# PrimeIntellect-ai/pi-quant

Measured on AMD Instinct MI355X. Metric: GiB/s quantize fp32->uint8 (numel=27.26M, nearest), higher is better.
Workload: dtype f32

## Files before the change

pi-quant_amd/csrc/quant_kernels.hpp:

```cpp
#pragma once

#include <cstdio>
#include <cstdlib>

#include "device_math.hpp"
#include "stop_event.hpp"

namespace pq {

typedef uint32_t u32x4 __attribute__((ext_vector_type(4)));
typedef uint32_t u32x2 __attribute__((ext_vector_type(2)));

enum : int { ST_PLAIN = 0, ST_NT = 1, ST_WT = 2 };
constexpr int mem_policy(bool nt_loads, int store_policy) { return (nt_loads ? 1 : 0) | (store_policy << 1); }

template <bool NT, typename T>
__device__ __forceinline__ T ld(const T* p) {
    typedef T unaligned_t __attribute__((aligned(1)));
    const unaligned_t* q = reinterpret_cast<const unaligned_t*>(p);
    if constexpr (NT) return __builtin_nontemporal_load(q);
    else return *q;
}

template <int POLICY, typename T>
__device__ __forceinline__ void st(T* p, T v) {
    typedef T unaligned_t __attribute__((aligned(1)));
    if constexpr (POLICY == ST_NT) {
        __builtin_nontemporal_store(v, reinterpret_cast<unaligned_t*>(p));
    } else if constexpr (POLICY == ST_WT) {
        if constexpr (sizeof(T) == 16) asm volatile("global_store_dwordx4 %0, %1, off sc0 sc1\n\ts_nop 1" ::"v"(p), "v"(v) : "memory");
        else if constexpr (sizeof(T) == 8) asm volatile("global_store_dwordx2 %0, %1, off sc0 sc1\n\ts_nop 0" ::"v"(p), "v"(v) : "memory");
        else if constexpr (sizeof(T) == 4) asm volatile("global_store_dword %0, %1, off sc0 sc1" ::"v"(p), "v"(v) : "memory");
        else if constexpr (sizeof(T) == 2) asm volatile("global_store_short %0, %1, off sc0 sc1" ::"v"(p), "v"(static_cast<uint32_t>(v)) : "memory");
        else asm volatile("global_store_byte %0, %1, off sc0 sc1" ::"v"(p), "v"(static_cast<uint32_t>(v)) : "memory");
    } else {
        *reinterpret_cast<unaligned_t*>(p) = v;
    }
}

template <int DT_IN>
struct InVec {
    static constexpr int EPV = DT_IN == DT_F32 ? 4 : 8;
    static __device__ __forceinline__ void unpack(const u32x4& raw, float (&v)[EPV]) {
        if constexpr (DT_IN == DT_F32) {
#pragma unroll
            for (int e = 0; e < 4; ++e) v[e] = __uint_as_float(raw[e]);
        } else {
#pragma unroll
            for (int e = 0; e < 4; ++e) {
                v[2 * e] = __uint_as_float(raw[e] << 16);
                v[2 * e + 1] = __uint_as_float(raw[e] & 0xffff0000u);
            }
        }
    }
    static __device__ __forceinline__ float load_scalar(const void* in, int64_t i) {
        if constexpr (DT_IN == DT_F32) return static_cast<const float*>(in)[i];
        else return bf16_bits_to_f32(static_cast<const uint16_t*>(in)[i]);
    }
};

template <int BITS>
struct QuantRefBlock {
    static constexpr int value = BITS == 8 ? 64 : 16;
};

template <int DT_IN, int BITS, int MODE>
__device__ __forceinline__ void quantize_bytes_guarded(const void* in, uint8_t* out, int64_t numel, int64_t byte_begin,
                                                       int64_t byte_end, const QuantParams& p, int64_t tid,
                                                       int64_t nthreads) {
    constexpr int PACK = 8 / BITS;
    constexpr int QMAX = (1 << BITS) - 1;
    for (int64_t b = byte_begin + tid; b < byte_end; b += nthreads) {
        [[maybe_unused]] RefPart part {};
        if constexpr (MODE == RM_NEAREST_FAST) {
            if (p.ref.on) part = ref_part<PACK, QuantRefBlock<BITS>::value>(p.ref, ref_partition_index<PACK>(p.ref, p.ref.index0 + b * PACK));
        }
        uint32_t acc = 0;
#pragma unroll
        for (int k = 0; k < PACK; ++k) {
            const int64_t i = b * PACK + k;
            if (i >= numel) continue;
            const float x = InVec<DT_IN>::load_scalar(in, i);
            uint32_t q;
            bool scalar_form = false;
            if constexpr (MODE == RM_NEAREST_FAST) {
                const int64_t g = p.ref.index0 + i;
                scalar_form = p.ref.on && (g < part.head_end || g >= part.body_end);
            }
            if (scalar_form) q = quant_nearest_tail32<QMAX>(x, p);
            else q = quant_one<MODE, QMAX>(x, p, static_cast<uint64_t>(i));
            acc |= q << (k * BITS);
        }
        out[b] = static_cast<uint8_t>(acc);
    }
}

template <int DT_IN, int BITS, int MODE>
__global__ void __launch_bounds__(256) quantize_scalar_kernel(const void* in, uint8_t* out, int64_t numel, QuantParams p_arg) {
    const QuantParams p = resolved(p_arg);
    constexpr int PACK = 8 / BITS;
    const int64_t nbytes = (numel + PACK - 1) / PACK;
    quantize_bytes_guarded<DT_IN, BITS, MODE>(in, out, numel, 0, nbytes, p,
                                              static_cast<int64_t>(blockIdx.x) * blockDim.x + threadIdx.x,
                                              static_cast<int64_t>(gridDim.x) * blockDim.x);
}

template <int DT_IN, int BITS, int MODE>
__device__ __forceinline__ void quantize_vec(const u32x4& raw, const QuantParams& p, const ElementKeys& keys, uint64_t e0,
                                             uint32_t (&w)[(InVec<DT_IN>::EPV * BITS / 8) > 4 ? 2 : 1]) {
    constexpr int EPV = InVec<DT_IN>::EPV, QMAX = (1 << BITS) - 1, WORDS = (EPV * BITS / 8) > 4 ? 2 : 1;
    float v[EPV];
    InVec<DT_IN>::unpack(raw, v);
#pragma unroll
    for (int j = 0; j < WORDS; ++j) w[j] = 0;
    if constexpr (MODE == RM_NEAREST_FAST) {
#pragma unroll
        for (int e = 0; e < EPV; e += 2) {
            uint32_t q0, q1;
            quant_nearest_fast2<QMAX>(v[e], v[e + 1], p, q0, q1);
            w[(e * BITS) >> 5] |= (q0 | (q1 << BITS)) << ((e * BITS) & 31);
        }
    } else if constexpr (MODE == RM_STOCH_ELEM) {
#pragma unroll
        for (int e = 0; e < EPV; ++e) {
            const uint32_t q = quant_stochastic<QMAX>(v[e], p, element_threshold(keys, p.index_base + e0 + e));
            w[(e * BITS) >> 5] |= q << ((e * BITS) & 31);
        }
    } else {
#pragma unroll
        for (int e = 0; e < EPV; ++e) {
            const uint32_t q = quant_one<MODE, QMAX>(v[e], p, e0 + e);
            w[(e * BITS) >> 5] |= q << ((e * BITS) & 31);
        }
    }
}

__device__ __forceinline__ uint32_t bfi32(uint32_t mask, uint32_t a, uint32_t b) { return (a & mask) | (b & ~mask); }

template <int EPV>
__device__ __forceinline__ void pack_saturated_u8(const float (&tz)[EPV], uint32_t (&w)[EPV / 4]) {
#pragma unroll
    for (int j = 0; j < EPV / 4; ++j) {
        uint32_t acc = 0;
#pragma unroll
        for (int e = 0; e < 4; ++e) acc = __builtin_amdgcn_cvt_pk_u8_f32(tz[j * 4 + e], static_cast<uint32_t>(e), acc);
        w[j] = acc;
    }
}

template <int BITS, int EPV>
__device__ __forceinline__ void pack_normalised(const float (&tn)[EPV], uint32_t (&w)[(EPV * BITS / 8) > 4 ? 2 : 1]) {
    auto P = [](float a, float b) -> uint32_t {
        typedef unsigned short u16x2 __attribute__((ext_vector_type(2)));
        const u16x2 r = __builtin_amdgcn_cvt_pknorm_u16(a, b);
        return __builtin_bit_cast(uint32_t, r);
    };
    constexpr uint32_t LOW_BYTES = 0x06040200u;
    static_assert(BITS == 4 || BITS == 2, "8-bit outputs gain nothing from the normalised domain (one v_perm per four elements against nothing): pack_saturated_u8");
    if constexpr (BITS == 4) {
        if constexpr (EPV == 8) {
            const uint32_t even = __builtin_amdgcn_perm(P(tn[4], tn[6]), P(tn[0], tn[2]), LOW_BYTES);
            const uint32_t odd = __builtin_amdgcn_perm(P(tn[5], tn[7]), P(tn[1], tn[3]), LOW_BYTES);
            w[0] = bfi32(0x0f0f0f0fu, even, odd);
        } else {
            const uint32_t m = bfi32(0x0f0f0f0fu, P(tn[0], tn[2]), P(tn[1], tn[3]));
            w[0] = __builtin_amdgcn_perm(0u, m, 0x0c0c0200u);
        }
    } else {
        if constexpr (EPV == 8) {
            const uint32_t t1 = bfi32(0x33333333u, P(tn[0], tn[4]), P(tn[1], tn[5]));
            const uint32_t t2 = bfi32(0x33333333u, P(tn[2], tn[6]), P(tn[3], tn[7]));
            const uint32_t u = bfi32(0x0f0f0f0fu, t1, t2);
            w[0] = __builtin_amdgcn_perm(0u, u, 0x0c0c0200u);
        } else {
            const uint32_t t = bfi32(0x33333333u, P(tn[0], tn[2]), P(tn[1], tn[3]));
            w[0] = bfi32(0x0fu, t, t >> 16) & 0xffu;
        }
    }
}

template <int N>
__device__ __forceinline__ void add_half_abs_round_down(const float (&r)[N], float (&out)[N]) {
    static_assert(N == 4, "the generic step exists for fp32 inputs only: four elements per vector");
    asm volatile("s_setreg_imm32_b32 hwreg(HW_REG_MODE, 0, 2), 2\n"
                 "v_add_f32_e64 %0, |%4|, 0.5\nv_add_f32_e64 %1, |%5|, 0.5\nv_add_f32_e64 %2, |%6|, 0.5\nv_add_f32_e64 %3, |%7|, 0.5\n"
                 "s_setreg_imm32_b32 hwreg(HW_REG_MODE, 0, 2), 0"
                 : "=&v"(out[0]), "=&v"(out[1]), "=&v"(out[2]), "=&v"(out[3])
                 : "v"(r[0]), "v"(r[1]), "v"(r[2]), "v"(r[3]));
}

template <int BITS, int EPV>
__device__ __forceinline__ void clamp_and_pack(const float (&s)[EPV], const BoundedStep& b, uint32_t (&w)[(EPV * BITS / 8) > 4 ? 2 : 1]) {
#pragma clang fp contract(off)
    constexpr float R = 1.0f / static_cast<float>((1 << BITS) - 1);
    float tz[EPV];
#pragma unroll
    for (int e = 0; e < EPV; e += 2) {
        const f32x2 pair = {s[e], s[e + 1]};
        f32x2 sum;
        if constexpr (BITS == 8) sum = pair + b.zp_float;
        else sum = __builtin_elementwise_fma(pair, f32x2 {R, R}, f32x2 {b.zp_norm, b.zp_norm});
        tz[e] = sum[0];
        tz[e + 1] = sum[1];
    }
    if constexpr (BITS == 8) pack_saturated_u8<EPV>(tz, w);
    else pack_normalised<BITS, EPV>(tz, w);
}

template <int DT_IN, int BITS, bool GENERIC = false>
__device__ __forceinline__ void quantize_vec_bounded(const u32x4& raw, float inv_scale, const BoundedStep& b,
                                                     uint32_t (&w)[(InVec<DT_IN>::EPV * BITS / 8) > 4 ? 2 : 1]) {
#pragma clang fp contract(off)
    constexpr int EPV = InVec<DT_IN>::EPV;
    float v[EPV];
    InVec<DT_IN>::unpack(raw, v);
    float t[EPV];
    if constexpr (GENERIC) {
        float prods[EPV], sums[EPV];
#pragma unroll
        for (int e = 0; e < EPV; e += 2) {
            const f32x2 x = {v[e], v[e + 1]};
            const f32x2 prod = x * inv_scale;
            prods[e] = prod[0];
            prods[e + 1] = prod[1];
        }
        add_half_abs_round_down<EPV>(prods, sums);
#pragma unroll
        for (int e = 0; e < EPV; ++e) t[e] = __builtin_copysignf(__builtin_floorf(sums[e]), prods[e]);
    } else {
#pragma unroll
        for (int e = 0; e < EPV; e += 2) {
            const f32x2 x = {v[e], v[e + 1]};
            const f32x2 prod = x * inv_scale;
            const f32x2 half = {__builtin_copysignf(0.5f, prod[0]), __builtin_copysignf(0.5f, prod[1])};
            const f32x2 adj = prod + half;
            t[e] = __builtin_truncf(adj[0]);
            t[e + 1] = __builtin_truncf(adj[1]);
        }
    }
    clamp_and_pack<BITS, EPV>(t, b, w);
}

template <int N, bool UNIFORM>
__device__ __forceinline__ void sub_abs_round_up(const float (&r)[N], const float (&t)[N], float (&out)[N]) {
    static_assert(N == 4 || N == 8, "one 16-byte vector of fp32 or bf16");
#define PQ_RU_ON "s_setreg_imm32_b32 hwreg(HW_REG_MODE, 0, 2), 1\n"
#define PQ_RU_OFF "s_setreg_imm32_b32 hwreg(HW_REG_MODE, 0, 2), 0"
    if constexpr (N == 4 && UNIFORM) {
        asm volatile(PQ_RU_ON "v_sub_f32_e64 %0, |%4|, %8\nv_sub_f32_e64 %1, |%5|, %8\nv_sub_f32_e64 %2, |%6|, %8\nv_sub_f32_e64 %3, |%7|, %8\n" PQ_RU_OFF
                     : "=&v"(out[0]), "=&v"(out[1]), "=&v"(out[2]), "=&v"(out[3])
                     : "v"(r[0]), "v"(r[1]), "v"(r[2]), "v"(r[3]), "v"(t[0]));
    } else if constexpr (N == 4) {
        asm volatile(PQ_RU_ON "v_sub_f32_e64 %0, |%4|, %8\nv_sub_f32_e64 %1, |%5|, %9\nv_sub_f32_e64 %2, |%6|, %10\nv_sub_f32_e64 %3, |%7|, %11\n" PQ_RU_OFF
                     : "=&v"(out[0]), "=&v"(out[1]), "=&v"(out[2]), "=&v"(out[3])
                     : "v"(r[0]), "v"(r[1]), "v"(r[2]), "v"(r[3]), "v"(t[0]), "v"(t[1]), "v"(t[2]), "v"(t[3]));
    } else if constexpr (UNIFORM) {
        asm volatile(PQ_RU_ON "v_sub_f32_e64 %0, |%8|, %16\nv_sub_f32_e64 %1, |%9|, %16\nv_sub_f32_e64 %2, |%10|, %16\nv_sub_f32_e64 %3, |%11|, %16\n"
                     "v_sub_f32_e64 %4, |%12|, %16\nv_sub_f32_e64 %5, |%13|, %16\nv_sub_f32_e64 %6, |%14|, %16\nv_sub_f32_e64 %7, |%15|, %16\n" PQ_RU_OFF
                     : "=&v"(out[0]), "=&v"(out[1]), "=&v"(out[2]), "=&v"(out[3]), "=&v"(out[4]), "=&v"(out[5]), "=&v"(out[6]), "=&v"(out[7])
                     : "v"(r[0]), "v"(r[1]), "v"(r[2]), "v"(r[3]), "v"(r[4]), "v"(r[5]), "v"(r[6]), "v"(r[7]), "v"(t[0]));
    } else {
        asm volatile(PQ_RU_ON "v_sub_f32_e64 %0, |%8|, %16\nv_sub_f32_e64 %1, |%9|, %17\nv_sub_f32_e64 %2, |%10|, %18\nv_sub_f32_e64 %3, |%11|, %19\n"
                     "v_sub_f32_e64 %4, |%12|, %20\nv_sub_f32_e64 %5, |%13|, %21\nv_sub_f32_e64 %6, |%14|, %22\nv_sub_f32_e64 %7, |%15|, %23\n" PQ_RU_OFF
                     : "=&v"(out[0]), "=&v"(out[1]), "=&v"(out[2]), "=&v"(out[3]), "=&v"(out[4]), "=&v"(out[5]), "=&v"(out[6]), "=&v"(out[7])
                     : "v"(r[0]), "v"(r[1]), "v"(r[2]), "v"(r[3]), "v"(r[4]), "v"(r[5]), "v"(r[6]), "v"(r[7]), "v"(t[0]), "v"(t[1]), "v"(t[2]), "v"(t[3]), "v"(t[4]),
                       "v"(t[5]), "v"(t[6]), "v"(t[7]));
    }
#undef PQ_RU_ON
#undef PQ_RU_OFF
}

template <int DT_IN, int BITS, int MODE>
__device__ __forceinline__ void quantize_vec_bounded_stochastic(const u32x4& raw, const QuantParams& p, const ElementKeys& keys, uint64_t e0,
                                                                const BoundedStep& b, uint32_t (&w)[(InVec<DT_IN>::EPV * BITS / 8) > 4 ? 2 : 1]) {
#pragma clang fp contract(off)
    static_assert(MODE == RM_STOCH_CALL || MODE == RM_STOCH_ELEM, "stochastic modes only");
    constexpr int EPV = InVec<DT_IN>::EPV;
    float v[EPV];
    InVec<DT_IN>::unpack(raw, v);
    float s[EPV], r[EPV], tau[EPV], a[EPV];
#pragma unroll
    for (int e = 0; e < EPV; e += 2) {
        const f32x2 x = {v[e], v[e + 1]};
        const f32x2 prod = x * p.inv_scale;
        r[e] = prod[0];
        r[e + 1] = prod[1];
    }
#pragma unroll
    for (int e = 0; e < EPV; ++e) tau[e] = MODE == RM_STOCH_ELEM ? element_threshold(keys, p.index_base + e0 + e) : p.threshold;
    sub_abs_round_up<EPV, MODE == RM_STOCH_CALL>(r, tau, a);
#pragma unroll
    for (int e = 0; e < EPV; ++e) s[e] = __builtin_copysignf(__builtin_ceilf(a[e]), r[e]);
    clamp_and_pack<BITS, EPV>(s, b, w);
}

template <int DT_IN, int BITS, int MODE>
__device__ __forceinline__ void quantize_vec_short(const u32x4& raw, const QuantParams& p, const ElementKeys& keys, uint64_t e0, const BoundedStep& b,
                                                   uint32_t (&w)[(InVec<DT_IN>::EPV * BITS / 8) > 4 ? 2 : 1]) {
    if constexpr (MODE == RM_NEAREST_FAST || MODE == RM_NEAREST_I64) quantize_vec_bounded<DT_IN, BITS, MODE == RM_NEAREST_I64>(raw, p.inv_scale, b, w);
    else quantize_vec_bounded_stochastic<DT_IN, BITS, MODE>(raw, p, keys, e0, b, w);
}

template <int BITS>
__device__ __forceinline__ BoundedStep bounded_step_for(int32_t zp32) {
    constexpr float QMAX = static_cast<float>((1 << BITS) - 1);
    return BoundedStep {static_cast<float>(zp32), (static_cast<float>(zp32) + 0.3f * QMAX / 65535.0f) * (1.0f / QMAX)};
}

__device__ __forceinline__ float vec_absmax_f32(const u32x4& raw, float m, bool& nan) {
#pragma unroll
    for (int e = 0; e < 4; e += 2) {
        const float a = __uint_as_float(raw[e]), b = __uint_as_float(raw[e + 1]);
        m = __builtin_fmaxf(__builtin_fmaxf(__builtin_fabsf(a), __builtin_fabsf(b)), m);
        nan |= __builtin_isunordered(a, b);
    }
    return m;
}

typedef uint16_t u16x2 __attribute__((ext_vector_type(2)));
__device__ __forceinline__ uint32_t vec_absmax_bits_bf16(const u32x4& raw, uint32_t m) {
#pragma unroll
    for (int e = 0; e < 4; ++e)
        m = __builtin_bit_cast(uint32_t, __builtin_elementwise_max(__builtin_bit_cast(u16x2, m), __builtin_bit_cast(u16x2, raw[e] & 0x7fff7fffu)));
    return m;
}
__device__ __forceinline__ float absmax_bits_to_float(uint32_t m) { return __uint_as_float(max(m & 0xffffu, m >> 16) << 16); }

template <int OB, int POLICY>
__device__ __forceinline__ void store_packed(uint8_t* dst, const uint32_t (&w)[OB > 4 ? 2 : 1]) {
    if constexpr (OB == 1) st<POLICY>(dst, static_cast<uint8_t>(w[0]));
    else if constexpr (OB == 2) st<POLICY>(reinterpret_cast<uint16_t*>(dst), static_cast<uint16_t>(w[0]));
    else if constexpr (OB == 4) st<POLICY>(reinterpret_cast<uint32_t*>(dst), w[0]);
    else st<POLICY>(reinterpret_cast<u32x2*>(dst), u32x2 {w[0], w[1]});
}

struct QuantKernargs {
    const void* in;
    uint8_t* out;
    int64_t numel;
    uint64_t ref_m;
    float inv_scale;
    int32_t zp32;
    const ParamRecord* dyn;
    uint32_t flags, look_w;
    QuantParams p;
};
constexpr uint32_t kQuantKernargRef = static_cast<uint32_t>(__builtin_offsetof(QuantKernargs, p) + __builtin_offsetof(QuantParams, ref));

template <int DT_IN, int BITS, int U, int BLOCK>
struct QuantTile {
    static constexpr int EPV = InVec<DT_IN>::EPV;
    static constexpr int OB = EPV * BITS / 8;
    static constexpr int WAVES = BLOCK / 64;
    static constexpr int WAVE_VECS = U * 64;
    static constexpr int WAVE_OUT_BYTES = WAVE_VECS * OB;
    static constexpr int LANE_OUT_BYTES = U * OB;
    static constexpr int64_t BLOCK_ELEMS = static_cast<int64_t>(WAVES) * WAVE_VECS * EPV;
};

template <int DT_IN, int BITS, int MODE, int U, bool STAGE, int NT, int BLOCK>
__global__ void __launch_bounds__(BLOCK)
quantize_kernel(const void* __restrict__ in, uint8_t* __restrict__ out, int64_t numel, uint64_t look_m, float inv_scale, int32_t zp32,
                const ParamRecord* dyn, uint32_t flags, uint32_t look_w, QuantParams p_arg) {
    static_assert((QuantTile<DT_IN, BITS, U, BLOCK>::BLOCK_ELEMS & (QuantTile<DT_IN, BITS, U, BLOCK>::BLOCK_ELEMS - 1)) == 0, "a shift");
    const uint32_t tiles = static_cast<uint32_t>(static_cast<uint64_t>(numel) / static_cast<uint64_t>(QuantTile<DT_IN, BITS, U, BLOCK>::BLOCK_ELEMS));
    const int64_t n_tiles = tiles;
    const uint32_t tile_stride = tiles > 0 ? tiles : 1u;
    const int head = static_cast<int>(flags >> 16);
    [[maybe_unused]] const bool ref_on = MODE == RM_NEAREST_FAST && (flags & 2u) != 0;
    p_arg.inv_scale = inv_scale;
    p_arg.zp32 = zp32;
    p_arg.dyn = dyn;
    const QuantParams p = resolved(p_arg);
    using T = QuantTile<DT_IN, BITS, U, BLOCK>;
    constexpr int EPV = T::EPV, OB = T::OB;
    constexpr int WORDS = OB > 4 ? 2 : 1;
    constexpr bool NT_LD = (NT & 1) != 0;
    constexpr int NT_ST = NT >> 1;

    __shared__ __attribute__((aligned(16))) uint8_t lds[STAGE ? T::WAVES * T::WAVE_OUT_BYTES : 16];

    const int lane = threadIdx.x & 63;
    const int wave = __builtin_amdgcn_readfirstlane(threadIdx.x >> 6);
    const u32x4* __restrict__ in16 = static_cast<const u32x4*>(in);
    uint32_t zp_in_range = flags & 1u;
    if (dyn != nullptr) zp_in_range = dyn->zero_point >= 0 && dyn->zero_point <= (1 << BITS) - 1 ? 1u : 0u;
    const bool short_ok = zp_in_range != 0;
    const BoundedStep bstep = bounded_step_for<BITS>(p.zp32);
    const float abs_inv = __builtin_fabsf(p.inv_scale);

    if (blockIdx.x < tiles) {
        const int64_t tile = blockIdx.x;
        const int64_t v0 = (tile * T::WAVES + wave) * T::WAVE_VECS;

        u32x4 raw[U];
        if (DT_IN == DT_BF16 && (reinterpret_cast<uintptr_t>(in) & 2u) != 0) {
            const uint8_t* base = static_cast<const uint8_t*>(in) - 2;
#pragma unroll
            for (int k = 0; k < U; ++k) {
                const int64_t vec = v0 + k * 64 + lane;
                if ((vec == 0 && head == 0) || (vec + 1) * EPV >= numel) {
                    raw[k] = ld<NT_LD>(in16 + vec);
                    continue;
                }
                const uint8_t* a = base + vec * 16;
                const u32x4 t = ld<NT_LD>(reinterpret_cast<const u32x4*>(a));
                const uint32_t n = ld<NT_LD>(reinterpret_cast<const uint32_t*>(a + 16));
                raw[k] = u32x4 {__builtin_amdgcn_alignbit(t[1], t[0], 16), __builtin_amdgcn_alignbit(t[2], t[1], 16), __builtin_amdgcn_alignbit(t[3], t[2], 16),
                                __builtin_amdgcn_alignbit(n, t[3], 16)};
            }
        } else {
#pragma unroll
            for (int k = 0; k < U; ++k) raw[k] = ld<NT_LD>(in16 + v0 + k * 64 + lane);
        }

        [[maybe_unused]] int32_t ref_ta = 1, ref_tb = 0;
        [[maybe_unused]] RefSplit ref {};
        if constexpr (MODE == RM_NEAREST_FAST) {
            if (ref_on) {
                using Margins = RefMargins<8 / BITS, QuantRefBlock<BITS>::value>;
                const uint64_t wave_tile = static_cast<uint64_t>(tile) * T::WAVES + static_cast<uint32_t>(wave);
                bool look;
                if (look_m != 0) {
                    look = ref_first_look_fast<Margins::below>(look_m, look_w, static_cast<uint32_t>(wave_tile), T::WAVE_VECS * EPV);
                    if (look) ref = load_ref_split<kQuantKernargRef>();
                } else {
                    ref = load_ref_split<kQuantKernargRef>();
                    look = ref_first_look(ref, wave_tile);
                }
                if (look) {
                    const int64_t g0 = ref.index0 + v0 * EPV;
                    ref_candidates<8 / BITS, QuantRefBlock<BITS>::value>(ref, g0, g0 + static_cast<int64_t>(T::WAVE_VECS) * EPV, ref_ta, ref_tb);
                }
            }
        }

        [[maybe_unused]] ElementKeys keys {};
        if constexpr (MODE == RM_STOCH_ELEM) keys = element_keys_for(p, p.index_base + static_cast<uint64_t>(v0 + lane) * EPV);
        uint8_t* o = out + v0 * OB;
        auto put = [&](uint32_t (&w)[U][WORDS]) {
            if constexpr (!STAGE) {
#pragma unroll
                for (int k = 0; k < U; ++k) store_packed<OB, NT_ST>(o + static_cast<int64_t>(k * 64 + lane) * OB, w[k]);
            } else {
                uint8_t* s = lds + wave * T::WAVE_OUT_BYTES;
#pragma unroll
                for (int k = 0; k < U; ++k) {
                    uint8_t* dst = s + (k * 64 + lane) * OB;
                    if constexpr (OB == 1) *dst = static_cast<uint8_t>(w[k][0]);
                    else if constexpr (OB == 2) *reinterpret_cast<uint16_t*>(dst) = static_cast<uint16_t>(w[k][0]);
                    else if constexpr (OB == 4) *reinterpret_cast<uint32_t*>(dst) = w[k][0];
                    else *reinterpret_cast<u32x2*>(dst) = u32x2{w[k][0], w[k][1]};
                }
                __builtin_amdgcn_fence(__ATOMIC_RELEASE, "wavefront");
                __builtin_amdgcn_wave_barrier();
                __builtin_amdgcn_fence(__ATOMIC_ACQUIRE, "wavefront");
                if constexpr (T::LANE_OUT_BYTES >= 16) {
#pragma unroll
                    for (int j = 0; j < T::LANE_OUT_BYTES / 16; ++j) {
                        const u32x4 r = reinterpret_cast<const u32x4*>(s)[j * 64 + lane];
                        st<NT_ST>(reinterpret_cast<u32x4*>(o) + j * 64 + lane, r);
                    }
                } else if constexpr (T::LANE_OUT_BYTES == 8) {
                    st<NT_ST>(reinterpret_cast<u32x2*>(o) + lane, reinterpret_cast<const u32x2*>(s)[lane]);
                } else if constexpr (T::LANE_OUT_BYTES == 4) {
                    st<NT_ST>(reinterpret_cast<uint32_t*>(o) + lane, reinterpret_cast<const uint32_t*>(s)[lane]);
                } else {
                    st<NT_ST>(reinterpret_cast<uint16_t*>(o) + lane, reinterpret_cast<const uint16_t*>(s)[lane]);
                }
                __builtin_amdgcn_fence(__ATOMIC_RELEASE, "wavefront");
                __builtin_amdgcn_wave_barrier();
            }
        };
        bool ref_tile = false;
        if constexpr (MODE == RM_NEAREST_FAST) ref_tile = ref_ta <= ref_tb;
        if (__builtin_expect(ref_tile, 0)) {
            if constexpr (MODE == RM_NEAREST_FAST) {
                constexpr int QMAX = (1 << BITS) - 1;
                uint32_t m[U];
                ref_scalar_masks<8 / BITS, QuantRefBlock<BITS>::value, EPV, U>(ref, ref_ta, ref_tb, ref.index0 + (v0 + lane) * EPV, 64 * EPV, m);
                uint32_t w[U][WORDS];
#pragma unroll
                for (int k = 0; k < U; ++k) {
                    if (m[k] == 0) {
                        quantize_vec<DT_IN, BITS, MODE>(raw[k], p, keys, static_cast<uint64_t>(v0 + k * 64 + lane) * EPV, w[k]);
                        continue;
                    }
                    float v[EPV];
                    InVec<DT_IN>::unpack(raw[k], v);
#pragma unroll
                    for (int j = 0; j < WORDS; ++j) w[k][j] = 0;
#pragma unroll
                    for (int e = 0; e < EPV; ++e) {
                        const float prod = __fmul_rn(v[e], p.inv_scale);
                        const float r = ((m[k] >> e) & 1u) != 0 ? roundf(prod) : __fadd_rn(prod, __builtin_copysignf(0.5f, prod));
                        w[k][(e * BITS) >> 5] |= quant_nearest_finish<QMAX>(r, p) << ((e * BITS) & 31);
                    }
                }
                put(w);
            }
        } else {
            bool short_step = false;
            if (short_ok) {
                if (abs_inv < 5.0e8f) {
                    uint32_t o = 0;
    #pragma unroll
                    for (int k = 0; k < U; ++k) o |= raw[k][0] | raw[k][1] | raw[k][2] | raw[k][3];
                    short_step = __all((o & (DT_IN == DT_F32 ? 0x40000000u : 0x40004000u)) == 0 ? 1 : 0) != 0;
                }
                if (short_step) {
                } else if constexpr (DT_IN == DT_BF16) {
                    uint32_t m = 0;
    #pragma unroll
                    for (int k = 0; k < U; ++k) m = vec_absmax_bits_bf16(raw[k], m);
                    short_step = __all(__fmul_rn(absmax_bits_to_float(m), abs_inv) < 1.0e9f ? 1 : 0) != 0;
                } else {
                    float amax = 0.0f;
                    bool nan = false;
    #pragma unroll
                    for (int k = 0; k < U; ++k) amax = vec_absmax_f32(raw[k], amax, nan);
                    short_step = __all(!nan && __fmul_rn(amax, abs_inv) < 1.0e9f ? 1 : 0) != 0;
                }
            }
            if (__builtin_expect(short_step, 1)) {
                uint32_t w[U][WORDS];
#pragma unroll
                for (int k = 0; k < U; ++k) quantize_vec_short<DT_IN, BITS, MODE>(raw[k], p, keys, static_cast<uint64_t>(v0 + k * 64 + lane) * EPV, bstep, w[k]);
                put(w);
            } else {
                uint32_t w[U][WORDS];
#pragma unroll
                for (int k = 0; k < U; ++k) quantize_vec<DT_IN, BITS, MODE>(raw[k], p, keys, static_cast<uint64_t>(v0 + k * 64 + lane) * EPV, w[k]);
                put(w);
            }
        }
    }

    constexpr int PACK = 8 / BITS;
    const bool ragged = n_tiles * T::BLOCK_ELEMS < numel;
    if (ragged || head > 0) {
        const int64_t gtid = static_cast<int64_t>(blockIdx.x) * BLOCK + threadIdx.x, gthreads = static_cast<int64_t>(tile_stride) * BLOCK;
        const int64_t rag_bytes = ragged ? (numel + PACK - 1) / PACK - n_tiles * T::BLOCK_ELEMS / PACK : 0, head_bytes = head / PACK;
        if (static_cast<int64_t>(blockIdx.x) * BLOCK + wave * 64 >= (rag_bytes > head_bytes ? rag_bytes : head_bytes)) return;
        QuantParams pg = p;
        pg.ref = RefSplit {};
        if constexpr (MODE == RM_NEAREST_FAST) {
            if (ref_on) pg.ref = load_ref_split<kQuantKernargRef>();
        }
        if (ragged) quantize_bytes_guarded<DT_IN, BITS, MODE>(in, out, numel, n_tiles * T::BLOCK_ELEMS / PACK, (numel + PACK - 1) / PACK, pg, gtid, gthreads);
        if (head > 0) {
            QuantParams ph = pg;
            ph.index_base -= static_cast<uint64_t>(head);
            ph.ref.index0 -= head;
            quantize_bytes_guarded<DT_IN, BITS, MODE>(static_cast<const uint8_t*>(in) - static_cast<int64_t>(head) * (DT_IN == DT_F32 ? 4 : 2), out - head / PACK,
                                                      head, 0, head / PACK, ph, gtid, gthreads);
        }
    }
}

template <int DT_IN, int BITS, int MODE, int U, bool STAGE, int NT, int BLOCK>
inline void launch_quantize_kernel(hipStream_t stream, const void* in, uint8_t* out, int64_t numel, int64_t n_tiles, const QuantParams& p, int head) {
    using Tile = QuantTile<DT_IN, BITS, U, BLOCK>;
    const uint32_t flags = (p.zp64 >= 0 && p.zp64 <= (1 << BITS) - 1 ? 1u : 0u) | (p.ref.on ? 2u : 0u) | (static_cast<uint32_t>(head) << 16);
    if (n_tiles > 0x7fffffff) {
        fprintf(stderr, "quantize: %lld tiles in one launch\n", static_cast<long long>(n_tiles));
        abort();
    }
    const RefFastLook look = MODE == RM_NEAREST_FAST ? ref_fast_look_constants(p.ref, Tile::BLOCK_ELEMS / Tile::WAVES, 8 / BITS, QuantRefBlock<BITS>::value) : RefFastLook {0, 0};
    if (n_tiles != numel / Tile::BLOCK_ELEMS) {
        fprintf(stderr, "quantize: %lld tiles for %lld elements\n", static_cast<long long>(n_tiles), static_cast<long long>(numel));
        abort();
    }
    const unsigned grid = n_tiles > 0 ? static_cast<unsigned>(n_tiles) : 1u;
    PQ_LAUNCH((quantize_kernel<DT_IN, BITS, MODE, U, STAGE, NT, BLOCK>), dim3(grid), dim3(BLOCK), 0, stream, in, out, numel, look.m, p.inv_scale, p.zp32, p.dyn, flags,
              look.w, p);
}

}
```

Baseline: 4511.

## Add lean fp32->u8 nearest kernel with compile-time edge and reference specialization

Splits the quantize kernel into a device function templated on whether edge handling is needed and on the reference-check mode. A lean kernel with a smaller argument list serves fp32->uint8 nearest when no reference is active. The hot path is reordered to issue loads first, resolve parameters lazily, and end the program right after the short-step store, so per-block scalar setup and tail logic are skipped. This cuts per-wave overhead in a bandwidth-bound kernel but adds more template variants and inline asm ordering barriers.

```diff
diff --git a/pi-quant_amd/csrc/quant_kernels.hpp b/pi-quant_amd/csrc/quant_kernels.hpp
--- a/pi-quant_amd/csrc/quant_kernels.hpp
+++ b/pi-quant_amd/csrc/quant_kernels.hpp
@@ -2,6 +2,7 @@
 
 #include <cstdio>
 #include <cstdlib>
+#include <type_traits>
 
 #include "device_math.hpp"
 #include "stop_event.hpp"
@@ -346,6 +347,19 @@
     QuantParams p;
 };
 constexpr uint32_t kQuantKernargRef = static_cast<uint32_t>(__builtin_offsetof(QuantKernargs, p) + __builtin_offsetof(QuantParams, ref));
+using QuantKernelFn = void (*)(decltype(QuantKernargs::in), decltype(QuantKernargs::out), decltype(QuantKernargs::numel), decltype(QuantKernargs::ref_m),
+                               decltype(QuantKernargs::inv_scale), decltype(QuantKernargs::zp32), decltype(QuantKernargs::dyn), decltype(QuantKernargs::flags),
+                               decltype(QuantKernargs::look_w), decltype(QuantKernargs::p));
+static_assert(sizeof(QuantKernargs) == 184 && kQuantKernargRef == 104, "nine leading scalars (14 dwords) and the parameter struct");
+
+enum : int { REF_OFF = 0, REF_FLAG = 1, REF_ON = 2 };
+
+#ifndef PQ_STAMP
+#define PQ_STAMP_DECL()
+#define PQ_STAMP(i)
+#define PQ_STAMP_DATA()
+#define PQ_STAMP_END()
+#endif
 
 template <int DT_IN, int BITS, int U, int BLOCK>
 struct QuantTile {
@@ -358,38 +372,42 @@
     static constexpr int64_t BLOCK_ELEMS = static_cast<int64_t>(WAVES) * WAVE_VECS * EPV;
 };
 
-template <int DT_IN, int BITS, int MODE, int U, bool STAGE, int NT, int BLOCK>
-__global__ void __launch_bounds__(BLOCK)
-quantize_kernel(const void* __restrict__ in, uint8_t* __restrict__ out, int64_t numel, uint64_t look_m, float inv_scale, int32_t zp32,
-                const ParamRecord* dyn, uint32_t flags, uint32_t look_w, QuantParams p_arg) {
+template <int DT_IN, int BITS, int MODE, int U, bool STAGE, int NT, int BLOCK, bool EDGES, int REF>
+__device__ __forceinline__ void quantize_tiles(const void* __restrict__ in, uint8_t* __restrict__ out, int64_t numel, uint64_t look_m, float inv_scale, int32_t zp32,
+                                               const ParamRecord* dyn, uint32_t flags, uint32_t look_w, const QuantParams& p_arg) {
     static_assert((QuantTile<DT_IN, BITS, U, BLOCK>::BLOCK_ELEMS & (QuantTile<DT_IN, BITS, U, BLOCK>::BLOCK_ELEMS - 1)) == 0, "a shift");
-    const uint32_t tiles = static_cast<uint32_t>(static_cast<uint64_t>(numel) / static_cast<uint64_t>(QuantTile<DT_IN, BITS, U, BLOCK>::BLOCK_ELEMS));
-    const int64_t n_tiles = tiles;
-    const uint32_t tile_stride = tiles > 0 ? tiles : 1u;
-    const int head = static_cast<int>(flags >> 16);
-    [[maybe_unused]] const bool ref_on = MODE == RM_NEAREST_FAST && (flags & 2u) != 0;
-    p_arg.inv_scale = inv_scale;
-    p_arg.zp32 = zp32;
-    p_arg.dyn = dyn;
-    const QuantParams p = resolved(p_arg);
     using T = QuantTile<DT_IN, BITS, U, BLOCK>;
     constexpr int EPV = T::EPV, OB = T::OB;
     constexpr int WORDS = OB > 4 ? 2 : 1;
     constexpr bool NT_LD = (NT & 1) != 0;
     constexpr int NT_ST = NT >> 1;
+    constexpr int PACK = 8 / BITS;
+    constexpr int REF_MODE = MODE == RM_NEAREST_FAST ? REF : REF_OFF;
+    constexpr uint32_t kEdgeBlocks = static_cast<uint32_t>(((T::BLOCK_ELEMS / PACK > 128 ? T::BLOCK_ELEMS / PACK : 128) + BLOCK - 1) / BLOCK);
 
     __shared__ __attribute__((aligned(16))) uint8_t lds[STAGE ? T::WAVES * T::WAVE_OUT_BYTES : 16];
 
+    PQ_STAMP_DECL();
+    PQ_STAMP(0);
     const int lane = threadIdx.x & 63;
     const int wave = __builtin_amdgcn_readfirstlane(threadIdx.x >> 6);
     const u32x4* __restrict__ in16 = static_cast<const u32x4*>(in);
-    uint32_t zp_in_range = flags & 1u;
-    if (dyn != nullptr) zp_in_range = dyn->zero_point >= 0 && dyn->zero_point <= (1 << BITS) - 1 ? 1u : 0u;
-    const bool short_ok = zp_in_range != 0;
-    const BoundedStep bstep = bounded_step_for<BITS>(p.zp32);
-    const float abs_inv = __builtin_fabsf(p.inv_scale);
-
-    if (blockIdx.x < tiles) {
+    auto parameters = [&](uint32_t& zp_in_range) {
+        QuantParams p = p_arg;
+        p.inv_scale = inv_scale;
+        p.zp32 = zp32;
+        p.dyn = dyn;
+        zp_in_range = flags & 1u;
+        if (__builtin_expect(dyn != nullptr, 0)) {
+            p = resolved(p);
+            zp_in_range = p.zp64 >= 0 && p.zp64 <= (1 << BITS) - 1 ? 1u : 0u;
+        }
+        return p;
+    };
+    [[maybe_unused]] uint32_t tiles = 0;
+    if constexpr (EDGES) tiles = static_cast<uint32_t>(static_cast<uint64_t>(numel) / static_cast<uint64_t>(T::BLOCK_ELEMS));
+
+    if (!EDGES || blockIdx.x < tiles) {
         const int64_t tile = blockIdx.x;
         const int64_t v0 = (tile * T::WAVES + wave) * T::WAVE_VECS;
 
@@ -399,7 +417,7 @@
 #pragma unroll
             for (int k = 0; k < U; ++k) {
                 const int64_t vec = v0 + k * 64 + lane;
-                if ((vec == 0 && head == 0) || (vec + 1) * EPV >= numel) {
+                if ((vec == 0 && (flags >> 16) == 0) || (vec + 1) * EPV >= numel) {
                     raw[k] = ld<NT_LD>(in16 + vec);
                     continue;
                 }
@@ -414,25 +432,20 @@
             for (int k = 0; k < U; ++k) raw[k] = ld<NT_LD>(in16 + v0 + k * 64 + lane);
         }
 
-        [[maybe_unused]] int32_t ref_ta = 1, ref_tb = 0;
-        [[maybe_unused]] RefSplit ref {};
-        if constexpr (MODE == RM_NEAREST_FAST) {
-            if (ref_on) {
-                using Margins = RefMargins<8 / BITS, QuantRefBlock<BITS>::value>;
-                const uint64_t wave_tile = static_cast<uint64_t>(tile) * T::WAVES + static_cast<uint32_t>(wave);
-                bool look;
-                if (look_m != 0) {
-                    look = ref_first_look_fast<Margins::below>(look_m, look_w, static_cast<uint32_t>(wave_tile), T::WAVE_VECS * EPV);
-                    if (look) ref = load_ref_split<kQuantKernargRef>();
-                } else {
-                    ref = load_ref_split<kQuantKernargRef>();
-                    look = ref_first_look(ref, wave_tile);
-                }
-                if (look) {
-                    const int64_t g0 = ref.index0 + v0 * EPV;
-                    ref_candidates<8 / BITS, QuantRefBlock<BITS>::value>(ref, g0, g0 + static_cast<int64_t>(T::WAVE_VECS) * EPV, ref_ta, ref_tb);
-                }
-            }
+        asm volatile("" ::: "memory");
+        PQ_STAMP(1);
+        uint32_t zp_in_range;
+        const QuantParams p = parameters(zp_in_range);
+        const bool short_ok = zp_in_range != 0;
+        const BoundedStep bstep = bounded_step_for<BITS>(p.zp32);
+        const float abs_inv = __builtin_fabsf(p.inv_scale);
+
+        [[maybe_unused]] bool look = false;
+        if constexpr (REF_MODE != REF_OFF) {
+            using Margins = RefMargins<8 / BITS, QuantRefBlock<BITS>::value>;
+            const uint32_t wave_tile = static_cast<uint32_t>(tile) * T::WAVES + static_cast<uint32_t>(wave);
+            const bool ref_on = REF_MODE == REF_ON || (flags & 2u) != 0;
+            look = ref_on & ((look_m == 0) | ref_first_look_fast<Margins::below>(look_m, look_w, wave_tile, T::WAVE_VECS * EPV));
         }
 
         [[maybe_unused]] ElementKeys keys {};
@@ -472,10 +485,52 @@
                 __builtin_amdgcn_wave_barrier();
             }
         };
+        auto short_step_and_store = [&](const QuantParams& pp) {
+            uint32_t w[U][WORDS];
+#pragma unroll
+            for (int k = 0; k < U; ++k) quantize_vec_short<DT_IN, BITS, MODE>(raw[k], pp, keys, static_cast<uint64_t>(v0 + k * 64 + lane) * EPV, bstep, w[k]);
+            put(w);
+        };
+        bool done = false;
+        PQ_STAMP_DATA();
+        int below_two = 0;
+        if (__builtin_expect(!look, 1)) {
+            uint32_t bits = 0;
+            asm volatile("" : "+v"(bits));
+#pragma unroll
+            for (int k = 0; k < U; ++k) bits |= raw[k][0] | raw[k][1] | raw[k][2] | raw[k][3];
+            below_two = __all((bits & (DT_IN == DT_F32 ? 0x40000000u : 0x40004000u)) == 0 ? 1 : 0);
+        }
+        if (__builtin_expect((static_cast<int>(!look) & static_cast<int>(short_ok) & static_cast<int>(abs_inv < 5.0e8f) & (below_two != 0 ? 1 : 0)) != 0, 1)) {
+            QuantParams hot = p;
+            asm volatile("" : "+v"(hot.inv_scale));
+            short_step_and_store(hot);
+            PQ_STAMP(3);
+            PQ_STAMP_END();
+            if constexpr (!EDGES) {
+                asm volatile("s_endpgm");
+                return;
+            } else if (__builtin_expect(blockIdx.x >= kEdgeBlocks, 1)) {
+                __builtin_amdgcn_endpgm();
+            }
+            done = true;
+        }
+        [[maybe_unused]] int32_t ref_ta = 1, ref_tb = 0;
+        [[maybe_unused]] RefSplit ref {};
+        if constexpr (REF_MODE != REF_OFF) {
+            if (!done && look) {
+                ref = load_ref_split<kQuantKernargRef>();
+                if (look_m != 0 || ref_first_look(ref, static_cast<uint64_t>(tile) * T::WAVES + static_cast<uint32_t>(wave))) {
+                    const int64_t g0 = ref.index0 + v0 * EPV;
+                    ref_candidates<8 / BITS, QuantRefBlock<BITS>::value>(ref, g0, g0 + static_cast<int64_t>(T::WAVE_VECS) * EPV, ref_ta, ref_tb);
+                }
+            }
+        }
         bool ref_tile = false;
-        if constexpr (MODE == RM_NEAREST_FAST) ref_tile = ref_ta <= ref_tb;
-        if (__builtin_expect(ref_tile, 0)) {
-            if constexpr (MODE == RM_NEAREST_FAST) {
+        if constexpr (REF_MODE != REF_OFF) ref_tile = ref_ta <= ref_tb;
+        if (done) {
+        } else if (ref_tile) {
+            if constexpr (REF_MODE != REF_OFF) {
                 constexpr int QMAX = (1 << BITS) - 1;
                 uint32_t m[U];
                 ref_scalar_masks<8 / BITS, QuantRefBlock<BITS>::value, EPV, U>(ref, ref_ta, ref_tb, ref.index0 + (v0 + lane) * EPV, 64 * EPV, m);
@@ -502,31 +557,21 @@
         } else {
             bool short_step = false;
             if (short_ok) {
-                if (abs_inv < 5.0e8f) {
-                    uint32_t o = 0;
-    #pragma unroll
-                    for (int k = 0; k < U; ++k) o |= raw[k][0] | raw[k][1] | raw[k][2] | raw[k][3];
-                    short_step = __all((o & (DT_IN == DT_F32 ? 0x40000000u : 0x40004000u)) == 0 ? 1 : 0) != 0;
-                }
-                if (short_step) {
-                } else if constexpr (DT_IN == DT_BF16) {
+                if constexpr (DT_IN == DT_BF16) {
                     uint32_t m = 0;
-    #pragma unroll
+#pragma unroll
                     for (int k = 0; k < U; ++k) m = vec_absmax_bits_bf16(raw[k], m);
                     short_step = __all(__fmul_rn(absmax_bits_to_float(m), abs_inv) < 1.0e9f ? 1 : 0) != 0;
                 } else {
                     float amax = 0.0f;
                     bool nan = false;
-    #pragma unroll
+#pragma unroll
                     for (int k = 0; k < U; ++k) amax = vec_absmax_f32(raw[k], amax, nan);
                     short_step = __all(!nan && __fmul_rn(amax, abs_inv) < 1.0e9f ? 1 : 0) != 0;
                 }
             }
-            if (__builtin_expect(short_step, 1)) {
-                uint32_t w[U][WORDS];
-#pragma unroll
-                for (int k = 0; k < U; ++k) quantize_vec_short<DT_IN, BITS, MODE>(raw[k], p, keys, static_cast<uint64_t>(v0 + k * 64 + lane) * EPV, bstep, w[k]);
-                put(w);
+            if (short_step) {
+                short_step_and_store(p);
             } else {
                 uint32_t w[U][WORDS];
 #pragma unroll
@@ -536,16 +581,21 @@
         }
     }
 
-    constexpr int PACK = 8 / BITS;
+    if constexpr (!EDGES) return;
+    if (blockIdx.x >= kEdgeBlocks) return;
+    const int head = static_cast<int>(flags >> 16);
+    const int64_t n_tiles = tiles;
+    const uint32_t tile_stride = tiles > 0 ? tiles : 1u;
     const bool ragged = n_tiles * T::BLOCK_ELEMS < numel;
     if (ragged || head > 0) {
         const int64_t gtid = static_cast<int64_t>(blockIdx.x) * BLOCK + threadIdx.x, gthreads = static_cast<int64_t>(tile_stride) * BLOCK;
         const int64_t rag_bytes = ragged ? (numel + PACK - 1) / PACK - n_tiles * T::BLOCK_ELEMS / PACK : 0, head_bytes = head / PACK;
         if (static_cast<int64_t>(blockIdx.x) * BLOCK + wave * 64 >= (rag_bytes > head_bytes ? rag_bytes : head_bytes)) return;
-        QuantParams pg = p;
+        uint32_t zp_in_range;
+        QuantParams pg = parameters(zp_in_range);
         pg.ref = RefSplit {};
-        if constexpr (MODE == RM_NEAREST_FAST) {
-            if (ref_on) pg.ref = load_ref_split<kQuantKernargRef>();
+        if constexpr (REF_MODE != REF_OFF) {
+            if (REF_MODE == REF_ON || (flags & 2u) != 0) pg.ref = load_ref_split<kQuantKernargRef>();
         }
         if (ragged) quantize_bytes_guarded<DT_IN, BITS, MODE>(in, out, numel, n_tiles * T::BLOCK_ELEMS / PACK, (numel + PACK - 1) / PACK, pg, gtid, gthreads);
         if (head > 0) {
@@ -558,7 +608,22 @@
     }
 }
 
-template <int DT_IN, int BITS, int MODE, int U, bool STAGE, int NT, int BLOCK>
+template <int DT_IN, int BITS, int MODE, int U, bool STAGE, int NT, int BLOCK, bool EDGES = true, int REF = REF_FLAG>
+__global__ void __launch_bounds__(BLOCK)
+quantize_kernel(const void* __restrict__ in, uint8_t* __restrict__ out, int64_t numel, uint64_t look_m, float inv_scale, int32_t zp32,
+                const ParamRecord* dyn, uint32_t flags, uint32_t look_w, QuantParams p_arg) {
+    quantize_tiles<DT_IN, BITS, MODE, U, STAGE, NT, BLOCK, EDGES, REF>(in, out, numel, look_m, inv_scale, zp32, dyn, flags, look_w, p_arg);
+}
+
+template <int DT_IN, int BITS, int MODE, int U, bool STAGE, int NT, int BLOCK, bool EDGES>
+__global__ void __launch_bounds__(BLOCK)
+quantize_lean_kernel(const void* __restrict__ in, uint8_t* __restrict__ out, int64_t numel, float inv_scale, int32_t zp32, const ParamRecord* dyn, uint32_t flags) {
+    static_assert(MODE == RM_NEAREST_FAST, "the other steps read the 64-bit zero point, the threshold or the seed");
+    const QuantParams none {};
+    quantize_tiles<DT_IN, BITS, MODE, U, STAGE, NT, BLOCK, EDGES, REF_OFF>(in, out, numel, 0, inv_scale, zp32, dyn, flags, 0, none);
+}
+
+template <int DT_IN, int BITS, int MODE, int U, bool STAGE, int NT, int BLOCK, bool LEAN = (DT_IN == DT_F32 && BITS == 8 && MODE == RM_NEAREST_FAST)>
 inline void launch_quantize_kernel(hipStream_t stream, const void* in, uint8_t* out, int64_t numel, int64_t n_tiles, const QuantParams& p, int head) {
     using Tile = QuantTile<DT_IN, BITS, U, BLOCK>;
     const uint32_t flags = (p.zp64 >= 0 && p.zp64 <= (1 << BITS) - 1 ? 1u : 0u) | (p.ref.on ? 2u : 0u) | (static_cast<uint32_t>(head) << 16);
@@ -572,8 +637,26 @@
         abort();
     }
     const unsigned grid = n_tiles > 0 ? static_cast<unsigned>(n_tiles) : 1u;
-    PQ_LAUNCH((quantize_kernel<DT_IN, BITS, MODE, U, STAGE, NT, BLOCK>), dim3(grid), dim3(BLOCK), 0, stream, in, out, numel, look.m, p.inv_scale, p.zp32, p.dyn, flags,
-              look.w, p);
-}
-
-}
+#define PQ_QUANT_FULL(EDGES, REF)                                                                                                                              \
+    do {                                                                                                                                                       \
+        static_assert(std::is_same_v<decltype(&quantize_kernel<DT_IN, BITS, MODE, U, STAGE, NT, BLOCK, EDGES, REF>), QuantKernelFn>, "QuantKernargs");          \
+        PQ_LAUNCH((quantize_kernel<DT_IN, BITS, MODE, U, STAGE, NT, BLOCK, EDGES, REF>), dim3(grid), dim3(BLOCK), 0, stream, in, out, numel, look.m, p.inv_scale, \
+                  p.zp32, p.dyn, flags, look.w, p);                                                                                                            \
+    } while (0)
+    if constexpr (LEAN) {
+        const bool edges = head != 0 || n_tiles == 0 || n_tiles * Tile::BLOCK_ELEMS != numel;
+        if (p.ref.on) {
+            if (edges) PQ_QUANT_FULL(true, REF_ON);
+            else PQ_QUANT_FULL(false, REF_ON);
+        } else if (edges) {
+            PQ_LAUNCH((quantize_lean_kernel<DT_IN, BITS, MODE, U, STAGE, NT, BLOCK, true>), dim3(grid), dim3(BLOCK), 0, stream, in, out, numel, p.inv_scale, p.zp32, p.dyn, flags);
+        } else {
+            PQ_LAUNCH((quantize_lean_kernel<DT_IN, BITS, MODE, U, STAGE, NT, BLOCK, false>), dim3(grid), dim3(BLOCK), 0, stream, in, out, numel, p.inv_scale, p.zp32, p.dyn, flags);
+        }
+    } else {
+        PQ_QUANT_FULL(true, REF_FLAG);
+    }
+#undef PQ_QUANT_FULL
+}
+
+}
```

Result: no change. 4527, median of 6 (+0.4%).
